# videolan/dav1d

Hardware: AMD Instinct MI355X
Metric: reconstructed luma Mpixels/s (8K 4:2:0 10-bit) on the itx+mc recon path; bit-exact vs C (higher is better)
Workload: dtype int32; 1 GPU; frame_contexts=2, picture_layout=tiled, parity=not checked in this run (bench.py --full checks it)

## Files before the change

### dav1d_amd/csrc/api_recon.hip

```cpp
#include "lists.h"
#include <stdio.h>
#include <stdlib.h>
#include <new>
#include <algorithm>


int recon_fuse_mask(const Dav1dHipContext *c) { return c->recon_fuse & 31; }

extern "C" {

int dav1d_hip_recon_list_create(Dav1dHipContext *c, Dav1dHipReconList **out, const Dav1dHipPicture *geometry,
                                const Dav1dHipMcTask *mc, size_t n_mc, const Dav1dHipCompTask *comp, size_t n_comp,
                                const Dav1dHipItxTask *itx, size_t n_itx) {
    if (!c || !out || !geometry) return -EINVAL;
    *out = nullptr;
    if ((!itx && n_itx) || n_itx > 0xffffffffu) return -EINVAL;
    for (size_t i = 0; i < n_itx; i++) if (!itx_task_ok(itx[i])) return -EINVAL;
    Dav1dHipReconList *l = new (std::nothrow) Dav1dHipReconList();
    if (!l) return -ENOMEM;
    const Dav1dHipItxTask *const itx_all = itx;
    const size_t n_itx_all = n_itx;
    l->inter = nullptr; l->itx = nullptr; l->wide_ok = false;
    for (int k = 0; k < 5; k++) { l->f_tiles[k] = nullptr; l->f_tasks[k] = nullptr; l->f_n[k] = 0; }
    l->f_max_ref = 0;
// ... 92 lines not shown

void dav1d_hip_recon_list_destroy(Dav1dHipContext *c, Dav1dHipReconList *l) {
    if (!l) return;
    if (l->inter) dav1d_hip_inter_list_destroy(c, l->inter);
    if (l->itx) dav1d_hip_itx_list_destroy(c, l->itx);
    hipStreamSynchronize(c->stream);
    for (int k = 0; k < 5; k++) { if (l->f_tiles[k]) hipFree(l->f_tiles[k]); if (l->f_tasks[k]) hipFree(l->f_tasks[k]); }
    delete l;
}

static int recon_list_run_impl(Dav1dHipContext *c, const Dav1dHipReconList *l, const Dav1dHipPicture *dst, const Dav1dHipPicture *refs, int n_refs,
                               int16_t *prep, uint8_t *mask, void *coef, const bool wide, const DevPlanes *dst_twin) {
    if (!c || !l || !dst || !refs) return -EINVAL;
    const int bps = dst->bpc > 8 ? 2 : 1;
    for (int p = 0; p < 3; p++)
        if (l->stride_px[p] && dst->p[p].stride / bps != l->stride_px[p]) return -EINVAL;
    size_t n_paired = 0;
    bool paired_on_side = false;
    int n_ps = 0;
    for (int k = 0; k < 5; k++) n_paired += l->f_n[k];
    if (n_paired) {
        const DevPlanes dp = dev_planes(dst);
        DevPlanes rp[8];
        if (const int rv = checked_ref_planes(c, dst, refs, n_refs, l->f_max_ref, rp)) return rv;
        const bool side = c->concurrent && n_paired >= 16384;
        int rc = 0, lane = 0;
        n_ps = side ? std::max(1, std::min(3, c->recon_pair_streams)) : 0;
        if (side) {
            (void) hipEventRecord(c->ev_fork, c->stream);
            for (int j = 0; j < n_ps; j++) (void) hipStreamWaitEvent(c->side[c->recon_pair_first + j], c->ev_fork, 0);
        }
        for (int k = 4; k >= 0 && !rc; k--)
            if (l->f_n[k]) {
                const bool on_main = side && k == 0;
                rc = dav1d_hip_launch_recon_fused_out(&dp, rp, n_refs, dst->bpc, k, l->f_tiles[k], l->f_tasks[k], (int) l->f_n[k], prep, coef, c->recon_coop_below,
                                                      wide, dst_twin, side && !on_main ? c->side[c->recon_pair_first + lane] : c->stream);
                if (!on_main && n_ps) lane = (lane + 1) % n_ps;
            }
        for (int j = 0; j < n_ps; j++) (void) hipEventRecord(c->ev_pair[j], c->side[c->recon_pair_first + j]);
        if (rc) return rc;
        paired_on_side = side;
        if (!l->inter->mc->n && !l->inter->comp->n && !l->itx->n) {
            for (int j = 0; j < n_ps; j++) (void) hipStreamWaitEvent(c->stream, c->ev_pair[j], 0);
            return 0;
        }
    }
    const Dav1dHipMcList *ml = l->inter->mc;
    const long min_tasks = c->recon_pipeline;
    auto join_paired = [&]() {
        if (paired_on_side) for (int j = 0; j < n_ps; j++) (void) hipStreamWaitEvent(c->stream, c->ev_pair[j], 0);
    };
    if (!dst_twin && (min_tasks < 0 || !c->concurrent || mc_fused_min_bin() < MC_BINS || (long) l->itx->n < min_tasks)) {
        int rc = dav1d_hip_inter_list_run(c, l->inter, dst, refs, n_refs, prep, mask);
        if (!rc) rc = dav1d_hip_itx_list_run(c, l->itx, dst, coef);
        join_paired();
        return rc;
    }
    const DevPlanes dp = dev_planes(dst);
    DevPlanes rp[8];
    if (const int rv = checked_ref_planes(c, dst, refs, n_refs, ml->n ? ml->max_ref : 0, rp)) { join_paired(); return rv; }
    int rc = mc_regroup(c, const_cast<Dav1dHipMcList *>(ml), rp, n_refs);
    if (rc) { join_paired(); return rc; }
    const int n_lanes = paired_on_side ? 1
                      : std::max(1, std::min((int) Dav1dHipContext::N_SIDE, c->recon_lanes));
    hipStream_t sm = c->stream;
    (void) hipEventRecord(c->ev_fork, sm);
    for (int i = 0; i < n_lanes; i++) (void) hipStreamWaitEvent(c->side[i], c->ev_fork, 0);
// ... 154 lines not shown
```

### dav1d_amd/csrc/capi.h

```cpp
#pragma once
#include "common.h"
#include <errno.h>
#include <mutex>
#include <vector>

struct Dav1dHipContext {
    int device;
    hipStream_t stream;
    bool own_stream;
    void *scratch;
    size_t scratch_size;
    enum { N_SIDE = 6 };
    hipStream_t side[N_SIDE];
    hipEvent_t ev_fork, ev_join[N_SIDE];
    hipEvent_t ev_pair[3];
    hipEvent_t ev_bin[16];
    bool concurrent;
    int flow_min_steps;
    int flow_mode;
    int flow_groups;
    int intra_sb;
    int intra_sb_flow;
    int intra_sb_lds;
    int intra_sb_waves;
    long intra_sb_fallbacks;
    int intra_sb_one_below;
    int recon_fuse;
    long recon_pipeline;
    int recon_lanes;
    int chunk_upload;
    int recon_coop_below;
    int post_bands;
    int colour_cells;
    int recon_pair_streams;
    int recon_pair_first;
    hipStream_t pad_streams[8]; int n_pad_streams;
    int ref_twin;
    bool cdef_rows;
    bool cdef_full_copy;
    bool cdef_unit_kernel;
    hipEvent_t ev_t0, ev_t1;
    float last_ms;
    bool last_ms_pending;
    struct Slab { uint8_t *host; size_t cap; };
    std::mutex pool_mtx;
    std::vector<Slab> free_slabs[48];
    struct Arena { uint8_t *dev; size_t cap; };
    std::vector<Arena> free_arenas;
    std::vector<Arena> free_task_bufs;
    std::vector<Dav1dHipPicture> free_pictures;
    size_t arena_hint;
    uint32_t *band_cnt = nullptr, *band_flags = nullptr;
    uint32_t band_seq = 0;
    int chunk_hints;
    int prep_async;
    int chunk_order;
    size_t arena_min;
    size_t uarena_hint = 0;
    size_t carena_hint;
    uint8_t *gather_dev, *segtab_dev;
    size_t gather_cap, segtab_cap;
    uint8_t *pending_slab;
    size_t pending_slab_cap;
    hipStream_t copy_stream;
    hipEvent_t ev_copy;
    hipEvent_t ev_untile;
    hipEvent_t ev_retile;
// ... 347 lines not shown
```

### dav1d_amd/csrc/capi.hip

```cpp
#include "capi.h"

#ifndef RECON_FUSE_DEFAULT
#define RECON_FUSE_DEFAULT 15
#endif
#include <stdlib.h>
#include <string.h>
#include <atomic>
#include <new>
#include <algorithm>
extern "C" void dav1d_hip_note_context_device(int device);

extern "C" {


long long dav1d_hip_live[8];
int dav1d_hip_live_objects(long long out[4]) {
    if (!out) return -EINVAL;
    for (int i = 0; i < 4; i++) out[i] = __atomic_load_n(&dav1d_hip_live[i], __ATOMIC_RELAXED);
    return 0;
}

int dav1d_hip_open(Dav1dHipContext **out, int device, void *stream) {
    if (!out) return -EINVAL;
    *out = nullptr;
    int ndev = 0;
    if (hipGetDeviceCount(&ndev) != hipSuccess || ndev <= 0 || device < 0 || device >= ndev)
        return -ENODEV;
    if (hipSetDevice(device) != hipSuccess) return -ENODEV;
    Dav1dHipContext *c = new (std::nothrow) Dav1dHipContext();
    if (!c) return -ENOMEM;
    c->device = device;
    c->own_stream = stream == nullptr;
    dav1d_hip_note_context_device(device);
    c->scratch = nullptr;
    c->scratch_size = 0;
    if (stream) c->stream = (hipStream_t) stream;
    else if (hipStreamCreate(&c->stream) != hipSuccess) { delete c; return -ENODEV; }
#ifndef DAV1D_HIP_EMU
    {
        hipDeviceProp_t prop;
        if (hipGetDeviceProperties(&prop, device) != hipSuccess || strncmp(prop.gcnArchName, "gfx950", 6)) { delete c; return -ENODEV; }
    }
#endif
    auto env_int = [](const char *name, long dflt) { const char *e = getenv(name); return e ? atol(e) : dflt; };
    c->recon_fuse = (int) env_int("DAV1D_HIP_RECON_FUSE", RECON_FUSE_DEFAULT);
    c->recon_pipeline = env_int("DAV1D_HIP_RECON_PIPELINE", 16384);
    c->recon_lanes = (int) env_int("DAV1D_HIP_RECON_LANES", 1);
    c->chunk_upload = (int) env_int("DAV1D_HIP_CHUNK_UPLOAD", 0);
    c->recon_coop_below = (int) env_int("DAV1D_HIP_RECON_COOP_BELOW", 4096);
    c->post_bands = (int) env_int("DAV1D_HIP_POST_BANDS", 0);
    c->colour_cells = (int) env_int("DAV1D_HIP_COLOUR_CELLS", 0);
    c->ref_twin = (int) env_int("DAV1D_HIP_REF_TWIN", 1);
    c->recon_pair_streams = (int) env_int("DAV1D_HIP_RECON_PAIR_STREAMS", 2);
    static std::atomic<int> n_opened{0};
    const int ctx_index = n_opened.fetch_add(1);
    auto env_list = [&](const char *name, long dflt) {
        const char *e = getenv(name);
        if (!e || !*e) return dflt;
        int n = 1;
        for (const char *q = e; *q; q++) n += *q == ',';
        int want = ctx_index % n;
        const char *q = e;
        while (want-- > 0) q = strchr(q, ',') + 1;
        return atol(q);
    };
    c->recon_pair_first = (int) std::max(1L, std::min(3L, env_list("DAV1D_HIP_RECON_PAIR_FIRST", 2)));
    c->n_pad_streams = (int) std::max(0L, std::min(8L, env_list("DAV1D_HIP_STREAM_PAD", 1)));
    for (int i = 0; i < c->n_pad_streams; i++)
        if (hipStreamCreateWithFlags(&c->pad_streams[i], hipStreamNonBlocking) != hipSuccess) { c->n_pad_streams = i; break; }
    const char *ser = getenv("DAV1D_HIP_SERIAL");
    c->concurrent = !(ser && atoi(ser));
    const char *cu = getenv("DAV1D_HIP_CDEF_UNIT");
    c->cdef_unit_kernel = cu && atoi(cu);
    c->cdef_full_copy = env_int("DAV1D_HIP_FILTER_FULL_COPY", 0) != 0;
    c->cdef_rows = env_int("DAV1D_HIP_CDEF_ROWS", 1) != 0;
    const char *fg = getenv("DAV1D_HIP_FLOW_GROUPS");
    c->flow_groups = fg && atoi(fg) > 0 ? atoi(fg) : 512;
    const char *fm = getenv("DAV1D_HIP_FLOW_MODE");
    c->flow_mode = fm ? atoi(fm) : 0;
    const char *fs = getenv("DAV1D_HIP_FLOW_MIN_STEPS");
    c->flow_min_steps = fs ? atoi(fs) : 200;
    const char *isb = getenv("DAV1D_HIP_INTRA_SB");
    c->intra_sb = isb ? atoi(isb) : 2;
    c->intra_sb_waves = (int) env_int("DAV1D_HIP_INTRA_SB_WAVES", 0);
    c->intra_sb_one_below = (int) env_int("DAV1D_HIP_INTRA_SB_ONE_BELOW", 0);
    c->intra_sb_fallbacks = 0;
// ... 99 lines not shown
    if (!graph) return -EIO;
    Dav1dHipGraph *g = new (std::nothrow) Dav1dHipGraph();
    if (!g) { hipGraphDestroy(graph); return -ENOMEM; }
    g->graph = graph;
    g->nodes = 0;
    (void) hipGraphGetNodes(graph, nullptr, &g->nodes);
    const hipError_t e = hipGraphInstantiate(&g->exec, graph, nullptr, nullptr, 0);
    if (e != hipSuccess) { hipGraphDestroy(graph); delete g; return hip_rc(e); }
    *out = g;
    return 0;
}

int dav1d_hip_graph_launch(Dav1dHipContext *c, const Dav1dHipGraph *g) {
    if (!c || !g) return -EINVAL;
    return hip_rc(hipGraphLaunch(g->exec, c->stream));
}

size_t dav1d_hip_graph_nodes(const Dav1dHipGraph *g) { return g ? g->nodes : 0; }

void dav1d_hip_graph_destroy(Dav1dHipContext *c, Dav1dHipGraph *g) {
    if (!g) return;
    if (c) hipStreamSynchronize(c->stream);
    hipGraphExecDestroy(g->exec);
    hipGraphDestroy(g->graph);
    delete g;
}
int dav1d_hip_get_option(Dav1dHipContext *c, const char *name, long *value) {
    if (!c || !name || !value) return -EINVAL;
    if (!strcmp(name, "intra_sb_fallbacks")) *value = c->intra_sb_fallbacks;
    else if (!strcmp(name, "intra_sb_waves")) *value = c->intra_sb_waves;
    else if (!strcmp(name, "intra_sb_one_below")) *value = c->intra_sb_one_below;
    else if (!strcmp(name, "recon_fuse")) *value = c->recon_fuse;
    else if (!strcmp(name, "recon_pair_streams")) *value = c->recon_pair_streams;
    else if (!strcmp(name, "recon_pair_first")) *value = c->recon_pair_first;
    else if (!strcmp(name, "ref_twin")) *value = c->ref_twin;
    else return -EINVAL;
    return 0;
}
int dav1d_hip_set_option(Dav1dHipContext *c, const char *name, long value) {
    if (!c || !name) return -EINVAL;
    if (!strcmp(name, "recon_fuse")) c->recon_fuse = (int) value;
    else if (!strcmp(name, "recon_pipeline")) c->recon_pipeline = value;
    else if (!strcmp(name, "recon_lanes")) c->recon_lanes = (int) value;
    else if (!strcmp(name, "chunk_upload")) c->chunk_upload = (int) value;
    else if (!strcmp(name, "recon_coop_below")) c->recon_coop_below = (int) value;
    else if (!strcmp(name, "post_bands")) c->post_bands = (int) value;
    else if (!strcmp(name, "colour_cells")) c->colour_cells = value < 0 ? 0 : value > 64 ? 64 : (int) value;
    else if (!strcmp(name, "ref_twin")) c->ref_twin = (int) value;
    else if (!strcmp(name, "recon_pair_streams")) c->recon_pair_streams = (int) value;
    else if (!strcmp(name, "recon_pair_first")) c->recon_pair_first = (int) std::max(1L, std::min(3L, (long) value));
    else if (!strcmp(name, "serial")) c->concurrent = !value;
    else if (!strcmp(name, "cdef_unit")) c->cdef_unit_kernel = value != 0;
    else if (!strcmp(name, "filter_full_copy")) c->cdef_full_copy = value != 0;
    else if (!strcmp(name, "cdef_rows")) c->cdef_rows = value != 0;
    else if (!strcmp(name, "flow_groups")) c->flow_groups = value > 0 ? (int) value : c->flow_groups;
    else if (!strcmp(name, "flow_mode")) c->flow_mode = (int) value;
    else if (!strcmp(name, "flow_min_steps")) c->flow_min_steps = (int) value;
    else if (!strcmp(name, "intra_sb")) c->intra_sb = (int) value;
    else if (!strcmp(name, "intra_sb_waves")) c->intra_sb_waves = value >= 8 ? 8 : value >= 4 ? 4 : value == 1 ? 1 : 0;
    else if (!strcmp(name, "intra_sb_one_below")) c->intra_sb_one_below = value > 0 ? (int) value : 0;
    else if (!strcmp(name, "intra_sb_lds")) c->intra_sb_lds = value != 0;
    else if (!strcmp(name, "intra_sb_flow")) c->intra_sb_flow = value != 0;
    else if (!strcmp(name, "intra_sb_fine")) dav1d_hip_sbw_set_fine(value != 0);
    else if (!strcmp(name, "intra_sb_fail_at")) dav1d_hip_sbw_set_fail_at((int) value);
    else if (!strcmp(name, "prep_async")) c->prep_async = value < 0 ? 0 : value > 2 ? 2 : (int) value;
    else if (!strcmp(name, "chunk_order")) c->chunk_order = value != 0;
    else if (!strcmp(name, "chunk_hints")) c->chunk_hints = value != 0;
    else if (!strcmp(name, "chunk_arena_min")) { if (value < 4096) return -EINVAL; c->arena_min = (size_t) 1 << 12; while (c->arena_min < (size_t) value) c->arena_min <<= 1; c->arena_hint = 0; }
    else return -EINVAL;
    return 0;
}

const char *dav1d_hip_version(void) { return "dav1d_hip 0.1 (gfx950)"; }
float dav1d_hip_last_kernel_ms(Dav1dHipContext *c) {
    if (!c) return 0.f;
    if (c->last_ms_pending) {
        c->last_ms_pending = false;
        c->last_ms = 0.f;
        if (hipEventSynchronize(c->ev_t1) == hipSuccess) (void) hipEventElapsedTime(&c->last_ms, c->ev_t0, c->ev_t1);
    }
    return c->last_ms;
}
// ... 106 lines not shown
```

### dav1d_amd/csrc/itx1d.h

```cpp
#pragma once
#include <hip/hip_runtime.h>
#include "common.h"

namespace itx1d {

__device__ static constexpr int kCos128[65] = {
    4096, 4095, 4091, 4085, 4076, 4065, 4052, 4036, 4017, 3996, 3973, 3948, 3920,
    3889, 3857, 3822, 3784, 3745, 3703, 3659, 3612, 3564, 3513, 3461, 3406, 3349,
    3290, 3229, 3166, 3102, 3035, 2967, 2896, 2824, 2751, 2675, 2598, 2520, 2440,
    2359, 2276, 2191, 2106, 2019, 1931, 1842, 1751, 1660, 1567, 1474, 1380, 1285,
    1189, 1092,  995,  897,  799,  700,  601,  501,  401,  301,  201,  101,    0,
};

__device__ constexpr int ilog2c(int v) { int r = 0; while (v > 1) { v >>= 1; r++; } return r; }
__device__ constexpr int brev(int v, int bits) {
    int r = 0;
    for (int i = 0; i < bits; i++) r |= ((v >> i) & 1) << (bits - 1 - i);
    return r;
}

__device__ __forceinline__ int clampi(int v, int lo, int hi) { return dv::clamp3(v, lo, hi); }

__device__ __forceinline__ int rot(int a, int b, int ka, int kb) {
    const int qa = ka > 2048 ? 1 : ka < -2048 ? -1 : 0;
    const int qb = kb > 2048 ? 1 : kb < -2048 ? -1 : 0;
    const int fa = ka - 4096 * qa, fb = kb - 4096 * qb;
    int acc = 2048;
    if (fb) acc = dv::mad_i24k(b, fb, acc);
    if (fa) acc = dv::mad_i24k(a, fa, acc);
    return (acc >> 12) + qa * a + qb * b;
}
__device__ __forceinline__ int rot45(int v) { return dv::mad_i24k(v, 181, 128) >> 8; }

template <int N>
__device__ __forceinline__ void idct(const int *in, int *out, const int lo, const int hi) {
    if constexpr (N == 2) {
        out[0] = rot45(in[0] + in[1]);
        out[1] = rot45(in[0] - in[1]);
    } else {
        constexpr int M = N / 2;
        int ev[M], e[M], t[M];
#pragma unroll
        for (int i = 0; i < M; i++) ev[i] = in[2 * i];
        idct<M>(ev, e, lo, hi);

        constexpr int bitsA = ilog2c(M / 2);
#pragma unroll
        for (int i = 0; i < M / 2; i++) {
            const int k = 4 * brev(i, bitsA) + 1;
            const int a = k * 64 / N;
            const int c = kCos128[a], s = kCos128[64 - a];
            const int x = in[k], y = in[N - k];
            t[i] = rot(x, y, s, -c);
            t[M - 1 - i] = rot(x, y, c, s);
        }
#pragma unroll
        for (int g = 2; g <= M / 2; g *= 2) {
#pragma unroll
            for (int G = 0; G < M / g; G++) {
#pragma unroll
                for (int i = 0; i < g / 2; i++) {
                    const int p = G * g + i, q = G * g + g - 1 - i;
                    const int u = t[p], v = t[q];
                    if (G & 1) { t[p] = clampi(v - u, lo, hi); t[q] = clampi(v + u, lo, hi); }
                    else       { t[p] = clampi(u + v, lo, hi); t[q] = clampi(u - v, lo, hi); }
                }
            }
            const int nblk = M / (4 * g) > 0 ? M / (4 * g) : 1;
            const int bitsR = ilog2c(nblk);
#pragma unroll
            for (int j = 0; j < M / 2; j++) {
                const int blk = j / (2 * g), o = j % (2 * g);
                if (o < g / 2 || o >= 3 * g / 2) continue;
                const int m = M - 1 - j;
                const int a = (4 * brev(blk, bitsR) + 1) * 64 * g / M;
                const int u = t[j], v = t[m];
                if (a == 32) {
                    t[j] = rot45(v - u);
                    t[m] = rot45(v + u);
                } else {
                    const int c = kCos128[a], s = kCos128[64 - a];
                    if (o < g) { t[j] = rot(v, u, s, -c);  t[m] = rot(v, u, c, s); }
                    else       { t[j] = rot(v, u, -c, -s); t[m] = rot(v, u, s, -c); }
                }
            }
        }
#pragma unroll
        for (int i = 0; i < M; i++) {
            const int u = e[i], v = t[M - 1 - i];
            out[i] = clampi(u + v, lo, hi);
            out[N - 1 - i] = clampi(u - v, lo, hi);
        }
    }
}

__device__ __forceinline__ void iadst4(const int *in, int *out) {
    const int a = in[0], b = in[1], c = in[2], d = in[3];
    using dv::mad_i24k;
    out[0] = (mad_i24k(a, 1321, mad_i24k(b, 3344 - 4096, mad_i24k(c, 3803 - 4096, mad_i24k(d, 2482 - 4096, 2048)))) >> 12)
             + b + c + d;
    out[1] = (mad_i24k(a, 2482 - 4096, mad_i24k(b, 3344 - 4096, mad_i24k(c, -1321, mad_i24k(d, -(3803 - 4096), 2048)))) >> 12)
             + a + b - d;
    out[2] = mad_i24k(a - c + d, 209, 128) >> 8;
    out[3] = (mad_i24k(a, 3803 - 4096, mad_i24k(b, -(3344 - 4096), mad_i24k(c, 2482 - 4096, mad_i24k(d, -1321, 2048)))) >> 12)
             + a - b + c;
}

template <int N>
__device__ __forceinline__ void iadst(const int *in, int *out, const int lo, const int hi) {
    static_assert(N == 8 || N == 16, "adst size");
    int t[N];
#pragma unroll
    for (int i = 0; i < N / 2; i++) {
        const int a = (4 * i + 1) * 32 / N;
        const int c = kCos128[a], s = kCos128[64 - a];
        const int x = in[N - 1 - 2 * i], y = in[2 * i];
        t[2 * i]     = rot(x, y, c, s);
        t[2 * i + 1] = rot(x, y, s, -c);
    }
// ... 68 lines not shown
```

### dav1d_amd/csrc/itx_body.h

```cpp
#pragma once
#include "common.h"
#include "itx1d.h"
#include "av1_scan_dev.h"
#include <type_traits>

namespace {

enum { K_DCT = 0, K_ADST = 1, K_IDENTITY = 2, K_FLIPADST = 3, K_WHT = 4 };

__host__ __device__ constexpr int tx_w(int tx) {
    constexpr int w[19] = { 4, 8, 16, 32, 64, 4, 8, 8, 16, 16, 32, 32, 64, 4, 16, 8, 32, 16, 64 };
    return w[tx];
}
__host__ __device__ constexpr int tx_h(int tx) {
    constexpr int h[19] = { 4, 8, 16, 32, 64, 8, 4, 16, 8, 32, 16, 64, 32, 16, 4, 32, 8, 64, 16 };
    return h[tx];
}
__host__ __device__ constexpr int tx_shift(int tx) {
    constexpr int s[19] = { 0, 1, 2, 2, 2, 0, 0, 1, 1, 1, 1, 1, 1, 1, 1, 2, 2, 2, 2 };
    return s[tx];
}
__host__ __device__ constexpr int cmin(int a, int b) { return a < b ? a : b; }
__host__ __device__ constexpr int cmax(int a, int b) { return a > b ? a : b; }

// ... 252 lines not shown
            dc = (dc + ((1 << SHIFT) >> 1)) >> SHIFT;
            dc = (dc * 181 + 128 + 2048) >> 12;
#pragma unroll
            for (int y = 0; y < H; y++)
                o[y * ostride] = ((pixel) dv::clamp3((int) dpx[y] + dc, 0, bitdepth_max));
        } else {
            int out[H];
            if (TX == 0 && wht) {
                if constexpr (H == 4) itx1d::iwht4(cin, out);
#pragma unroll
                for (int y = 0; y < H; y++)
                    o[y * ostride] = ((pixel) dv::clamp3((int) dpx[y] + out[y], 0, bitdepth_max));
            } else {
                tx1d<H>(k2, cin, col_min, col_max, [&](const int *res) {
                    if (k2 == K_FLIPADST) {
#pragma unroll
                        for (int y = 0; y < H; y++)
                            o[y * ostride] = ((pixel) dv::clamp3((int) dpx[y] + ((res[H - 1 - y] + 8) >> 4), 0, bitdepth_max));
                    } else {
#pragma unroll
                        for (int y = 0; y < H; y++)
                            o[y * ostride] = ((pixel) dv::clamp3((int) dpx[y] + ((res[y] + 8) >> 4), 0, bitdepth_max));
                    }
                });
            }
        }
    }
    DV_PHASE(PH + 3);
    DV_PHASE_WAVE(PH + 4);
}



template <int W, int H, int BPW, typename pixel>
__device__ __forceinline__ void tile_write_out(const pixel *tile, const Dav1dHipItxTask *__restrict__ tasks, const int nb,
                                               const DevPlanes &dst, const DevPlanes &twin, const bool has_twin, const bool raster = true,
                                               const uint32_t task_off = 0, const int task_plane = -1)
{
    constexpr int CP = W < 8 ? W : 8;
    constexpr int CPR = W / CP, PER_BLOCK = H * CPR, NCHK = BPW * PER_BLOCK;
    constexpr int BYTES = CP * (int) sizeof(pixel);
    typedef typename std::conditional<BYTES == 16, uint4, typename std::conditional<BYTES == 8, uint2, uint32_t>::type>::type piece_t;
    static_assert(BYTES == 4 || BYTES == 8 || BYTES == 16, "piece size");
    const int lane = dv::lane_id();
    constexpr int LPBX = 64 / BPW;
    constexpr bool OWN = BPW > 1 && PER_BLOCK == LPBX;
    constexpr bool ONE = BPW > 1 && PER_BLOCK % 64 == 0;
    constexpr bool TWO = BPW > 1 && PER_BLOCK == 32;
    const bool direct = task_plane >= 0 && (OWN || ONE || TWO);
    int bx = 0, by = 0, bpl = 0;
    if (direct) {
        if constexpr (OWN) {
            bpl = task_plane;
            dv::off_to_xy(task_off, bpl == 0 ? dst.stride[0] : bpl == 1 ? dst.stride[1] : dst.stride[2], bx, by);
        }
    } else if (task_plane >= 0) {
        const uint32_t off = BPW == 1 ? task_off : (uint32_t) __shfl((int) task_off, (lane & (BPW - 1)) * LPBX);
        bpl = BPW == 1 ? task_plane : __shfl(task_plane, (lane & (BPW - 1)) * LPBX);
        if (lane < nb) dv::off_to_xy(off, bpl == 0 ? dst.stride[0] : bpl == 1 ? dst.stride[1] : dst.stride[2], bx, by);
    } else if (lane < nb) {
        const Dav1dHipItxTask t = tasks[lane];
        bpl = t.plane;
        dv::off_to_xy(t.dst_off, bpl == 0 ? dst.stride[0] : bpl == 1 ? dst.stride[1] : dst.stride[2], bx, by);
    }
#pragma unroll
    for (int i0 = 0; i0 < NCHK; i0 += 64) {
        const int i = i0 + lane;
        const int b = BPW == 1 ? 0 : (i / PER_BLOCK) & (BPW - 1), rem = i - (i / PER_BLOCK) * PER_BLOCK;
        const int y = rem / CPR, c = rem - y * CPR;
        int x0, y0, pl;
        if constexpr (BPW == 1) { x0 = __builtin_amdgcn_readfirstlane(bx); y0 = __builtin_amdgcn_readfirstlane(by); pl = __builtin_amdgcn_readfirstlane(bpl); }
        else if (direct && OWN) { x0 = bx; y0 = by; pl = bpl; }
        else if (direct && ONE) {
            const int bl = ((i0 / PER_BLOCK) & (BPW - 1)) * LPBX;
            pl = dv::readlane(task_plane, bl);
            dv::off_to_xy((uint32_t) dv::readlane((int) task_off, bl), pl == 0 ? dst.stride[0] : pl == 1 ? dst.stride[1] : dst.stride[2], x0, y0);
        } else if (direct && TWO) {
            const int bl = ((i0 / PER_BLOCK) & (BPW - 1)) * LPBX;
            const bool hi = lane >= 32;
            pl = hi ? dv::readlane(task_plane, bl + LPBX) : dv::readlane(task_plane, bl);
            const uint32_t off = (uint32_t) (hi ? dv::readlane((int) task_off, bl + LPBX) : dv::readlane((int) task_off, bl));
            dv::off_to_xy(off, pl == 0 ? dst.stride[0] : pl == 1 ? dst.stride[1] : dst.stride[2], x0, y0);
        } else { x0 = __shfl(bx, b); y0 = __shfl(by, b); pl = __shfl(bpl, b); }
        if (i >= NCHK || i / PER_BLOCK >= nb) continue;
        const piece_t v = *reinterpret_cast<const piece_t *>(tile + b * itx_tile_stride(W, H) + y * W + c * CP);
#ifdef DV_KO_WRITE
        if (*reinterpret_cast<const uint32_t *>(&v) != 0xfeedbeefu) continue;
#endif
        const int X = x0 + c * CP, Y = y0 + y;
        const int stride = pl == 0 ? dst.stride[0] : pl == 1 ? dst.stride[1] : dst.stride[2];
        pixel *const base = reinterpret_cast<pixel *>(pl == 0 ? dst.data[0] : pl == 1 ? dst.data[1] : dst.data[2]);
        if (raster) *reinterpret_cast<piece_t *>(base + (dv::mul_i24(Y, stride) + X)) = v;
        if (has_twin) {
            pixel *const tb = reinterpret_cast<pixel *>(pl == 0 ? twin.data[0] : pl == 1 ? twin.data[1] : twin.data[2]);
            *reinterpret_cast<piece_t *>(tb + (dv::mul_i24(Y & ~7, stride) + ((X >> 3) << 6) + ((Y & 7) << 3) + (X & 7))) = v;
        }
    }
}

}
// ... 1 lines not shown
```

### dav1d_amd/csrc/recon.hip

```cpp
#define DV_UNIT recon
#include "mc_body.h"
#include "itx_body.h"
#include <string.h>

DV_PHASE_DEFINE(DV_UNIT)
namespace {

#ifndef RECON_WAVES
#define RECON_WAVES 7
#endif
#ifndef RECON_WAVES_8
#define RECON_WAVES_8 7
#endif
#ifndef RECON_WAVES_32
#define RECON_WAVES_32 7
#endif

constexpr int rc_log2(int v) { return v <= 1 ? 0 : 1 + rc_log2(v >> 1); }

template <int CLS> constexpr int recon_waves() {
    constexpr int W = 4 << CLS, TW = mc_cmin(W, 64), TH = mc_cmin(W, 16), TPB = (W / TW) * (W / TH);
    constexpr int LPB = cmax(cmin(W, 32), W), BPW = 64 / LPB, G = 64 / mc_cmin(64, TW * TH / 4);
    return (BPW * TPB + G - 1) / G;
}

template <int CLS, typename pixel, typename coef, bool COOP, bool TILED, bool WIDE>
__global__ __launch_bounds__(COOP ? 64 * recon_waves<CLS>() : 64, COOP ? 1 : CLS == 1 ? RECON_WAVES_8 : CLS == 3 ? RECON_WAVES_32 : RECON_WAVES)
void recon_fused_kernel(const DevPlanes dst, const RefSet refs, const McTile *__restrict__ tiles,
                        const Dav1dHipItxTask *__restrict__ tasks, const int n_blocks,
                        int16_t *__restrict__ prep, coef *__restrict__ cf, const int bitdepth_max, const DevPlanes twin)
{
    constexpr int TX = CLS;
    constexpr int W = 4 << CLS;
    constexpr int TW = mc_cmin(W, 64), TH = mc_cmin(W, 16);
    constexpr int TPB = (W / TW) * (W / TH);
    constexpr int LPB = cmax(cmin(W, 32), W), BPW = 64 / LPB;
    constexpr int G = 64 / mc_cmin(64, TW * TH / 4);
    constexpr int NW = COOP ? recon_waves<CLS>() : 1;
    constexpr int MC_B = (mc_lds_bytes<TW, TH, TILED>() + 15) / 16 * 16, PRED_B = BPW * itx_tile_stride(W, W) * (int) sizeof(pixel);
    constexpr int ITX_B = itx_lds_ints<TX>() * 4;
    constexpr int LDS_B = cmax(NW * MC_B + PRED_B, ITX_B);
    __shared__ uint4 smem[(LDS_B + 15) / 16];
    const int wave = NW == 1 ? 0 : (int) (threadIdx.x >> 6);
    uint4 *const smem_mc = reinterpret_cast<uint4 *>(reinterpret_cast<char *>(smem) + wave * MC_B);
    pixel *const pred = reinterpret_cast<pixel *>(reinterpret_cast<char *>(smem) + NW * MC_B);
    int *const smem_itx = reinterpret_cast<int *>(smem);

    const int group = (int) dv::xcd_chunk_id(blockIdx.x, gridDim.x);
    const int block0 = group * BPW;
    if (block0 >= n_blocks) return;
    DV_PHASE_BEGIN();
    const int nb = dv::imin(BPW, n_blocks - block0);
    const int tile0 = block0 * TPB, ntile = nb * TPB;
#ifdef DV_KO_NOMC
    if (bitdepth_max == 12345)
#endif
    if constexpr (NW == 1) {
        for (int c = 0; c < ntile; c += G) {
            mc_body<TW, TH, pixel, true, TILED>(dst, refs, tiles, tile0 + c, dv::imin(G, ntile - c), prep, bitdepth_max, smem_mc,
                                         pred, tile0, rc_log2(TPB), W, W);
            dv::wave_sync();
        }
    } else {
        const int c = wave * G;
        if (c < ntile)
            mc_body<TW, TH, pixel, true, TILED>(dst, refs, tiles, tile0 + c, dv::imin(G, ntile - c), prep, bitdepth_max, smem_mc,
                                         pred, tile0, rc_log2(TPB), W, W);
        __syncthreads();
        if (wave) return;
    }
    DV_PHASE(768 + CLS * 16 + 0);
    if constexpr (WIDE) {
        uint32_t toff = 0;
        int tpl = 0;
#ifdef DV_KO_NOITX
        if (bitdepth_max == 12345)
#endif
        itx_body<TX, pixel, coef, true, true>(dst, tasks, n_blocks, cf, bitdepth_max, group, smem_itx, pred, false, &toff, &tpl);
        dv::wave_sync();
        DV_PHASE(768 + CLS * 16 + 1);
#ifdef DV_KO_NOOUT
        if (bitdepth_max == 12345)
#endif
        tile_write_out<W, W, BPW, pixel>(pred, tasks + block0, nb, dst, twin, twin.data[0] != nullptr, twin.tiled != 2, toff, tpl);
        DV_PHASE(768 + CLS * 16 + 2);
    } else {
        itx_body<TX, pixel, coef, true>(dst, tasks, n_blocks, cf, bitdepth_max, group, smem_itx, pred);
        DV_PHASE(768 + CLS * 16 + 1);
    }
    DV_PHASE_WAVE(768 + CLS * 16 + 3);
}

template <int CLS, typename pixel, typename coef, bool TILED, bool WIDE>
void launch_cls(const DevPlanes &dst, const RefSet &refs, const McTile *tiles, const Dav1dHipItxTask *tasks, const int n,
                int16_t *prep, coef *cf, const int bitdepth_max, const int coop_below, const DevPlanes &twin, hipStream_t stream)
{
    constexpr int W = 4 << CLS, LPB = cmax(cmin(W, 32), W), BPW = 64 / LPB;
    const int groups = (n + BPW - 1) / BPW;
#ifndef DV_LEAN
    if (recon_waves<CLS>() > 1 && groups < coop_below)
        hipLaunchKernelGGL((recon_fused_kernel<CLS, pixel, coef, true, TILED, WIDE>), dim3(groups), dim3(64 * recon_waves<CLS>()), 0, stream,
                           dst, refs, tiles, tasks, n, prep, cf, bitdepth_max, twin);
    else
#endif
        hipLaunchKernelGGL((recon_fused_kernel<CLS, pixel, coef, false, TILED, WIDE>), dim3(groups), dim3(64), 0, stream,
                           dst, refs, tiles, tasks, n, prep, cf, bitdepth_max, twin);
}

template <typename pixel, typename coef, bool TILED, bool WIDE>
hipError_t launch_any(const int cls, const DevPlanes &dst, const RefSet &refs, const McTile *tiles, const Dav1dHipItxTask *tasks,
                      const int n, int16_t *prep, coef *cf, const int bitdepth_max, const int coop_below, const DevPlanes &twin, hipStream_t stream)
{
    switch (cls) {
    case 0: launch_cls<0, pixel, coef, TILED, WIDE>(dst, refs, tiles, tasks, n, prep, cf, bitdepth_max, coop_below, twin, stream); break;
    case 1: launch_cls<1, pixel, coef, TILED, WIDE>(dst, refs, tiles, tasks, n, prep, cf, bitdepth_max, coop_below, twin, stream); break;
    case 2: launch_cls<2, pixel, coef, TILED, WIDE>(dst, refs, tiles, tasks, n, prep, cf, bitdepth_max, coop_below, twin, stream); break;
    case 3: launch_cls<3, pixel, coef, TILED, WIDE>(dst, refs, tiles, tasks, n, prep, cf, bitdepth_max, coop_below, twin, stream); break;
    case 4: launch_cls<4, pixel, coef, TILED, WIDE>(dst, refs, tiles, tasks, n, prep, cf, bitdepth_max, coop_below, twin, stream); break;
    default: return hipErrorInvalidValue;
    }
    return hipGetLastError();
}

template <typename pixel, typename coef>
hipError_t launch_variant(const bool tiled, const bool wide, const int cls, const DevPlanes &dst, const RefSet &refs, const McTile *tiles,
                          const Dav1dHipItxTask *tasks, const int n, int16_t *prep, coef *cf, const int bitdepth_max, const int coop_below,
                          const DevPlanes &twin, hipStream_t st)
{
#ifdef DV_LEAN
    if (!tiled || !wide || sizeof(pixel) != 2) return hipErrorInvalidValue;
    if constexpr (sizeof(pixel) == 2) return launch_any<pixel, coef, true, true>(cls, dst, refs, tiles, tasks, n, prep, cf, bitdepth_max, coop_below, twin, st);
    else return hipErrorInvalidValue;
#else
    if (tiled) return wide ? launch_any<pixel, coef, true, true>(cls, dst, refs, tiles, tasks, n, prep, cf, bitdepth_max, coop_below, twin, st)
                           : launch_any<pixel, coef, true, false>(cls, dst, refs, tiles, tasks, n, prep, cf, bitdepth_max, coop_below, twin, st);
    return wide ? launch_any<pixel, coef, false, true>(cls, dst, refs, tiles, tasks, n, prep, cf, bitdepth_max, coop_below, twin, st)
                : launch_any<pixel, coef, false, false>(cls, dst, refs, tiles, tasks, n, prep, cf, bitdepth_max, coop_below, twin, st);
#endif
}
// ... 30 lines not shown
```

Measured before the change: 155,800 Mpixels/s.

## Add two-wave 64x64 recon-pair kernel splitting IDCT even/odd halves across waves

Adds a dedicated two-wave workgroup path for 64x64 inter+residual pairs (class 4). Each wave predicts half the tiles, then the 64-point row and column IDCTs are split so one wave computes the even half and the other the odd half, exchanging results through LDS. The kernel previously ran these as single-wave work with heavy per-lane register pressure. The change also turns on fuse bit 4 by default so this class is fused, and runs class 4 on the main stream instead of a side stream. It adds more barriers and LDS traffic per block.

Result: no change. 155,000 Mpixels/s (-0.5%).

```diff
diff --git a/dav1d_amd/csrc/api_recon.hip b/dav1d_amd/csrc/api_recon.hip
--- a/dav1d_amd/csrc/api_recon.hip
+++ b/dav1d_amd/csrc/api_recon.hip
@@ -148,7 +148,7 @@
         }
         for (int k = 4; k >= 0 && !rc; k--)
             if (l->f_n[k]) {
-                const bool on_main = side && k == 0;
+                const bool on_main = side && (k == 0 || (k == 4 && c->recon_pair64_main));
                 rc = dav1d_hip_launch_recon_fused_out(&dp, rp, n_refs, dst->bpc, k, l->f_tiles[k], l->f_tasks[k], (int) l->f_n[k], prep, coef, c->recon_coop_below,
                                                       wide, dst_twin, side && !on_main ? c->side[c->recon_pair_first + lane] : c->stream);
                 if (!on_main && n_ps) lane = (lane + 1) % n_ps;
diff --git a/dav1d_amd/csrc/capi.h b/dav1d_amd/csrc/capi.h
--- a/dav1d_amd/csrc/capi.h
+++ b/dav1d_amd/csrc/capi.h
@@ -33,6 +33,7 @@
     int post_bands;
     int colour_cells;
     int recon_pair_streams;
+    int recon_pair64_main;
     int recon_pair_first;
     hipStream_t pad_streams[8]; int n_pad_streams;
     int ref_twin;
diff --git a/dav1d_amd/csrc/capi.hip b/dav1d_amd/csrc/capi.hip
--- a/dav1d_amd/csrc/capi.hip
+++ b/dav1d_amd/csrc/capi.hip
@@ -1,7 +1,7 @@
 #include "capi.h"
 
 #ifndef RECON_FUSE_DEFAULT
-#define RECON_FUSE_DEFAULT 15
+#define RECON_FUSE_DEFAULT 31
 #endif
 #include <stdlib.h>
 #include <string.h>
@@ -52,6 +52,7 @@
     c->colour_cells = (int) env_int("DAV1D_HIP_COLOUR_CELLS", 0);
     c->ref_twin = (int) env_int("DAV1D_HIP_REF_TWIN", 1);
     c->recon_pair_streams = (int) env_int("DAV1D_HIP_RECON_PAIR_STREAMS", 2);
+    c->recon_pair64_main = (int) env_int("DAV1D_HIP_RECON_PAIR64_MAIN", 1);
     static std::atomic<int> n_opened{0};
     const int ctx_index = n_opened.fetch_add(1);
     auto env_list = [&](const char *name, long dflt) {
@@ -217,6 +218,7 @@
     else if (!strcmp(name, "intra_sb_one_below")) *value = c->intra_sb_one_below;
     else if (!strcmp(name, "recon_fuse")) *value = c->recon_fuse;
     else if (!strcmp(name, "recon_pair_streams")) *value = c->recon_pair_streams;
+    else if (!strcmp(name, "recon_pair64_main")) *value = c->recon_pair64_main;
     else if (!strcmp(name, "recon_pair_first")) *value = c->recon_pair_first;
     else if (!strcmp(name, "ref_twin")) *value = c->ref_twin;
     else return -EINVAL;
@@ -233,6 +235,7 @@
     else if (!strcmp(name, "colour_cells")) c->colour_cells = value < 0 ? 0 : value > 64 ? 64 : (int) value;
     else if (!strcmp(name, "ref_twin")) c->ref_twin = (int) value;
     else if (!strcmp(name, "recon_pair_streams")) c->recon_pair_streams = (int) value;
+    else if (!strcmp(name, "recon_pair64_main")) c->recon_pair64_main = value != 0;
     else if (!strcmp(name, "recon_pair_first")) c->recon_pair_first = (int) std::max(1L, std::min(3L, (long) value));
     else if (!strcmp(name, "serial")) c->concurrent = !value;
     else if (!strcmp(name, "cdef_unit")) c->cdef_unit_kernel = value != 0;
diff --git a/dav1d_amd/csrc/itx1d.h b/dav1d_amd/csrc/itx1d.h
--- a/dav1d_amd/csrc/itx1d.h
+++ b/dav1d_amd/csrc/itx1d.h
@@ -33,58 +33,73 @@
 __device__ __forceinline__ int rot45(int v) { return dv::mad_i24k(v, 181, 128) >> 8; }
 
 template <int N>
+__device__ __forceinline__ void idct(const int *in, int *out, const int lo, const int hi);
+
+template <int N>
+__device__ __forceinline__ void idct_even(const int *in, int *e, const int lo, const int hi) {
+    constexpr int M = N / 2;
+    int ev[M];
+#pragma unroll
+    for (int i = 0; i < M; i++) ev[i] = in[2 * i];
+    idct<M>(ev, e, lo, hi);
+}
+
+template <int N>
+__device__ __forceinline__ void idct_odd(const int *in, int *t, const int lo, const int hi) {
+    constexpr int M = N / 2;
+    constexpr int bitsA = ilog2c(M / 2);
+#pragma unroll
+    for (int i = 0; i < M / 2; i++) {
+        const int k = 4 * brev(i, bitsA) + 1;
+        const int a = k * 64 / N;
+        const int c = kCos128[a], s = kCos128[64 - a];
+        const int x = in[k], y = in[N - k];
+        t[i] = rot(x, y, s, -c);
+        t[M - 1 - i] = rot(x, y, c, s);
+    }
+#pragma unroll
+    for (int g = 2; g <= M / 2; g *= 2) {
+#pragma unroll
+        for (int G = 0; G < M / g; G++) {
+#pragma unroll
+            for (int i = 0; i < g / 2; i++) {
+                const int p = G * g + i, q = G * g + g - 1 - i;
+                const int u = t[p], v = t[q];
+                if (G & 1) { t[p] = clampi(v - u, lo, hi); t[q] = clampi(v + u, lo, hi); }
+                else       { t[p] = clampi(u + v, lo, hi); t[q] = clampi(u - v, lo, hi); }
+            }
+        }
+        const int nblk = M / (4 * g) > 0 ? M / (4 * g) : 1;
+        const int bitsR = ilog2c(nblk);
+#pragma unroll
+        for (int j = 0; j < M / 2; j++) {
+            const int blk = j / (2 * g), o = j % (2 * g);
+            if (o < g / 2 || o >= 3 * g / 2) continue;
+            const int m = M - 1 - j;
+            const int a = (4 * brev(blk, bitsR) + 1) * 64 * g / M;
+            const int u = t[j], v = t[m];
+            if (a == 32) {
+                t[j] = rot45(v - u);
+                t[m] = rot45(v + u);
+            } else {
+                const int c = kCos128[a], s = kCos128[64 - a];
+                if (o < g) { t[j] = rot(v, u, s, -c);  t[m] = rot(v, u, c, s); }
+                else       { t[j] = rot(v, u, -c, -s); t[m] = rot(v, u, s, -c); }
+            }
+        }
+    }
+}
+
+template <int N>
 __device__ __forceinline__ void idct(const int *in, int *out, const int lo, const int hi) {
     if constexpr (N == 2) {
         out[0] = rot45(in[0] + in[1]);
         out[1] = rot45(in[0] - in[1]);
     } else {
         constexpr int M = N / 2;
-        int ev[M], e[M], t[M];
-#pragma unroll
-        for (int i = 0; i < M; i++) ev[i] = in[2 * i];
-        idct<M>(ev, e, lo, hi);
-
-        constexpr int bitsA = ilog2c(M / 2);
-#pragma unroll
-        for (int i = 0; i < M / 2; i++) {
-            const int k = 4 * brev(i, bitsA) + 1;
-            const int a = k * 64 / N;
-            const int c = kCos128[a], s = kCos128[64 - a];
-            const int x = in[k], y = in[N - k];
-            t[i] = rot(x, y, s, -c);
-            t[M - 1 - i] = rot(x, y, c, s);
-        }
-#pragma unroll
-        for (int g = 2; g <= M / 2; g *= 2) {
-#pragma unroll
-            for (int G = 0; G < M / g; G++) {
-#pragma unroll
-                for (int i = 0; i < g / 2; i++) {
-                    const int p = G * g + i, q = G * g + g - 1 - i;
-                    const int u = t[p], v = t[q];
-                    if (G & 1) { t[p] = clampi(v - u, lo, hi); t[q] = clampi(v + u, lo, hi); }
-                    else       { t[p] = clampi(u + v, lo, hi); t[q] = clampi(u - v, lo, hi); }
-                }
-            }
-            const int nblk = M / (4 * g) > 0 ? M / (4 * g) : 1;
-            const int bitsR = ilog2c(nblk);
-#pragma unroll
-            for (int j = 0; j < M / 2; j++) {
-                const int blk = j / (2 * g), o = j % (2 * g);
-                if (o < g / 2 || o >= 3 * g / 2) continue;
-                const int m = M - 1 - j;
-                const int a = (4 * brev(blk, bitsR) + 1) * 64 * g / M;
-                const int u = t[j], v = t[m];
-                if (a == 32) {
-                    t[j] = rot45(v - u);
-                    t[m] = rot45(v + u);
-                } else {
-                    const int c = kCos128[a], s = kCos128[64 - a];
-                    if (o < g) { t[j] = rot(v, u, s, -c);  t[m] = rot(v, u, c, s); }
-                    else       { t[j] = rot(v, u, -c, -s); t[m] = rot(v, u, s, -c); }
-                }
-            }
-        }
+        int e[M], t[M];
+        idct_even<N>(in, e, lo, hi);
+        idct_odd<N>(in, t, lo, hi);
 #pragma unroll
         for (int i = 0; i < M; i++) {
             const int u = e[i], v = t[M - 1 - i];
diff --git a/dav1d_amd/csrc/itx_body.h b/dav1d_amd/csrc/itx_body.h
--- a/dav1d_amd/csrc/itx_body.h
+++ b/dav1d_amd/csrc/itx_body.h
@@ -308,11 +308,12 @@
 
 
 
-template <int W, int H, int BPW, typename pixel>
+template <int W, int H, int BPW, typename pixel, int NWV = 1>
 __device__ __forceinline__ void tile_write_out(const pixel *tile, const Dav1dHipItxTask *__restrict__ tasks, const int nb,
                                                const DevPlanes &dst, const DevPlanes &twin, const bool has_twin, const bool raster = true,
-                                               const uint32_t task_off = 0, const int task_plane = -1)
+                                               const uint32_t task_off = 0, const int task_plane = -1, const int wv = 0)
 {
+    static_assert(NWV == 1 || BPW == 1, "several waves share the tile of ONE block");
     constexpr int CP = W < 8 ? W : 8;
     constexpr int CPR = W / CP, PER_BLOCK = H * CPR, NCHK = BPW * PER_BLOCK;
     constexpr int BYTES = CP * (int) sizeof(pixel);
@@ -340,8 +341,8 @@
         dv::off_to_xy(t.dst_off, bpl == 0 ? dst.stride[0] : bpl == 1 ? dst.stride[1] : dst.stride[2], bx, by);
     }
 #pragma unroll
-    for (int i0 = 0; i0 < NCHK; i0 += 64) {
-        const int i = i0 + lane;
+    for (int i0 = 0; i0 < NCHK; i0 += 64 * NWV) {
+        const int i = i0 + (NWV == 1 ? 0 : wv * 64) + lane;
         const int b = BPW == 1 ? 0 : (i / PER_BLOCK) & (BPW - 1), rem = i - (i / PER_BLOCK) * PER_BLOCK;
         const int y = rem / CPR, c = rem - y * CPR;
         int x0, y0, pl;
diff --git a/dav1d_amd/csrc/recon.hip b/dav1d_amd/csrc/recon.hip
--- a/dav1d_amd/csrc/recon.hip
+++ b/dav1d_amd/csrc/recon.hip
@@ -1,6 +1,7 @@
 #define DV_UNIT recon
 #include "mc_body.h"
 #include "itx_body.h"
+#include "recon_pair64.h"
 #include <string.h>
 
 DV_PHASE_DEFINE(DV_UNIT)
@@ -19,6 +20,7 @@
 constexpr int rc_log2(int v) { return v <= 1 ? 0 : 1 + rc_log2(v >> 1); }
 
 template <int CLS> constexpr int recon_waves() {
+    if (CLS == 4) return 2;
     constexpr int W = 4 << CLS, TW = mc_cmin(W, 64), TH = mc_cmin(W, 16), TPB = (W / TW) * (W / TH);
     constexpr int LPB = cmax(cmin(W, 32), W), BPW = 64 / LPB, G = 64 / mc_cmin(64, TW * TH / 4);
     return (BPW * TPB + G - 1) / G;
@@ -41,6 +43,14 @@
     constexpr int ITX_B = itx_lds_ints<TX>() * 4;
     constexpr int LDS_B = cmax(NW * MC_B + PRED_B, ITX_B);
     __shared__ uint4 smem[(LDS_B + 15) / 16];
+    if constexpr (CLS == 4) {
+        static_assert(COOP && LDS_B == Pair64<pixel, coef, TILED>::LDS_B, "64x64 pairs: the two-wave workgroup");
+        const int block = (int) dv::xcd_chunk_id(blockIdx.x, gridDim.x);
+        if (block >= n_blocks) return;
+        DV_PHASE_BEGIN();
+        recon_pair64_body<pixel, coef, TILED, WIDE>(dst, refs, tiles, tasks, block, prep, cf, bitdepth_max, twin, smem);
+        DV_PHASE_WAVE(768 + CLS * 16 + 3);
+    } else {
     const int wave = NW == 1 ? 0 : (int) (threadIdx.x >> 6);
     uint4 *const smem_mc = reinterpret_cast<uint4 *>(reinterpret_cast<char *>(smem) + wave * MC_B);
     pixel *const pred = reinterpret_cast<pixel *>(reinterpret_cast<char *>(smem) + NW * MC_B);
@@ -89,6 +99,7 @@
         DV_PHASE(768 + CLS * 16 + 1);
     }
     DV_PHASE_WAVE(768 + CLS * 16 + 3);
+    }
 }
 
 template <int CLS, typename pixel, typename coef, bool TILED, bool WIDE>
@@ -97,14 +108,19 @@
 {
     constexpr int W = 4 << CLS, LPB = cmax(cmin(W, 32), W), BPW = 64 / LPB;
     const int groups = (n + BPW - 1) / BPW;
-#ifndef DV_LEAN
-    if (recon_waves<CLS>() > 1 && groups < coop_below)
+    if constexpr (CLS == 4) {
         hipLaunchKernelGGL((recon_fused_kernel<CLS, pixel, coef, true, TILED, WIDE>), dim3(groups), dim3(64 * recon_waves<CLS>()), 0, stream,
                            dst, refs, tiles, tasks, n, prep, cf, bitdepth_max, twin);
-    else
+    } else {
+#ifndef DV_LEAN
+        if (recon_waves<CLS>() > 1 && groups < coop_below)
+            hipLaunchKernelGGL((recon_fused_kernel<CLS, pixel, coef, true, TILED, WIDE>), dim3(groups), dim3(64 * recon_waves<CLS>()), 0, stream,
+                               dst, refs, tiles, tasks, n, prep, cf, bitdepth_max, twin);
+        else
 #endif
-        hipLaunchKernelGGL((recon_fused_kernel<CLS, pixel, coef, false, TILED, WIDE>), dim3(groups), dim3(64), 0, stream,
-                           dst, refs, tiles, tasks, n, prep, cf, bitdepth_max, twin);
+            hipLaunchKernelGGL((recon_fused_kernel<CLS, pixel, coef, false, TILED, WIDE>), dim3(groups), dim3(64), 0, stream,
+                               dst, refs, tiles, tasks, n, prep, cf, bitdepth_max, twin);
+    }
 }
 
 template <typename pixel, typename coef, bool TILED, bool WIDE>
diff --git a/dav1d_amd/csrc/recon_pair64.h b/dav1d_amd/csrc/recon_pair64.h
--- /dev/null
+++ b/dav1d_amd/csrc/recon_pair64.h
@@ -0,0 +1,175 @@
+#pragma once
+#include "mc_body.h"
+#include "itx_body.h"
+
+namespace {
+
+template <typename pixel, typename coef, bool TILED>
+struct Pair64 {
+    static constexpr int W = 64, SH = 32, TS = W + 1;
+    static constexpr int MC_B = (mc_lds_bytes<64, 16, TILED>() + 15) / 16 * 16;
+    static constexpr int PRED_B = itx_tile_stride(W, W) * (int) sizeof(pixel);
+    static constexpr int ROW_B = SH * TS * 4, SLAB_B = SH * SH * (int) sizeof(coef), XCH_B = 2 * 16 * 64 * 4;
+    static constexpr int LDS_B = 2 * MC_B + PRED_B;
+    static_assert(ROW_B % 16 == 0 && ROW_B + SLAB_B <= 2 * MC_B && XCH_B <= 2 * MC_B, "the transform's buffers fit the prediction windows");
+};
+
+template <typename pixel, typename coef, bool TILED, bool WIDE>
+__device__ __forceinline__ void recon_pair64_body(const DevPlanes &dst, const RefSet &refs, const McTile *__restrict__ tiles,
+                                                  const Dav1dHipItxTask *__restrict__ tasks, const int block, int16_t *__restrict__ prep,
+                                                  coef *__restrict__ cf, const int bitdepth_max, const DevPlanes &twin, uint4 *smem)
+{
+    typedef Pair64<pixel, coef, TILED> P;
+    constexpr int W = 64, SH = 32, TS = P::TS, SHIFT = tx_shift(4);
+    constexpr bool HBD = sizeof(pixel) == 2;
+    constexpr int NCH = P::SLAB_B / 16, NV = (NCH + 127) / 128;
+    const int tid = (int) threadIdx.x, lane = tid & 63;
+    const int wave = __builtin_amdgcn_readfirstlane(tid >> 6);
+
+    uint4 *const smem_mc = reinterpret_cast<uint4 *>(reinterpret_cast<char *>(smem) + wave * P::MC_B);
+    pixel *const pred = reinterpret_cast<pixel *>(reinterpret_cast<char *>(smem) + 2 * P::MC_B);
+    int *const tmp = reinterpret_cast<int *>(smem);
+    coef *const slab = reinterpret_cast<coef *>(reinterpret_cast<char *>(smem) + P::ROW_B);
+    int *const xch = reinterpret_cast<int *>(smem);
+
+    const Dav1dHipItxTask t = tasks[__builtin_amdgcn_readfirstlane(block)];
+    const bool dconly = t.txtp == 0 && t.eob < 1;
+    const bool packed = t.flags & DAV1D_HIP_ITX_PACKED;
+    coef *const gcf = cf + t.cf_off;
+    const int nch = dconly || packed ? 0 : (((int) t.rsv[0] | ((int) t.rsv[1] << 8)) * (int) sizeof(coef) + 15) >> 4;
+    const int tile0 = block * 4;
+#pragma unroll 1
+    for (int j = 0; j < 2; j++) {
+        mc_body<64, 16, pixel, true, TILED>(dst, refs, tiles, tile0 + 2 * wave + j, 1, prep, bitdepth_max, smem_mc, pred, tile0, 2, W, W);
+        dv::wave_sync();
+    }
+    int4 v[NV];
+#pragma unroll
+    for (int k = 0; k < NV; k++) {
+        v[k] = make_int4(0, 0, 0, 0);
+        if (tid + k * 128 < nch) v[k] = reinterpret_cast<const int4 *>(gcf)[tid + k * 128];
+    }
+    int dc = 0;
+    if (dconly) dc = gcf[0];
+    __syncthreads();
+
+    const int st0 = dst.stride[0], st1 = dst.stride[1], st2 = dst.stride[2];
+    void *const dp0 = dst.data[0], *const dp1 = dst.data[1], *const dp2 = dst.data[2];
+    const int stride = t.plane == 0 ? st0 : t.plane == 1 ? st1 : st2;
+    pixel *const d = reinterpret_cast<pixel *>(t.plane == 0 ? dp0 : t.plane == 1 ? dp1 : dp2) + t.dst_off + lane;
+    pixel *const pc = pred + lane;
+    auto emit = [&](const int y, const int res) {
+        const pixel px = (pixel) dv::clamp3((int) pc[y * W] + res, 0, bitdepth_max);
+        if (WIDE) pc[y * W] = px;
+        else d[y * stride] = px;
+    };
+
+    if (dconly) {
+        if (tid == 0 && !packed) gcf[0] = 0;
+        dc = (dc * 181 + 128) >> 8;
+        dc = (dc + ((1 << SHIFT) >> 1)) >> SHIFT;
+        dc = (dc * 181 + 128 + 2048) >> 12;
+#pragma unroll
+        for (int y = 0; y < 32; y++) emit(wave * 32 + y, dc);
+    } else {
+#pragma unroll
+        for (int k = 0; k < NV; k++) {
+            const int i = tid + k * 128;
+            if (i < NCH) reinterpret_cast<int4 *>(slab)[i] = v[k];
+            if (i < nch) reinterpret_cast<int4 *>(gcf)[i] = make_int4(0, 0, 0, 0);
+        }
+        if (packed) {
+            __syncthreads();
+            const int cls = (t.txtp == 11 || t.txtp == 13 || t.txtp == 15) ? 1 : (t.txtp == 10 || t.txtp == 12 || t.txtp == 14) ? 2 : 0;
+            const uint16_t *const scan = av1_scans + av1_scan_off[4];
+            for (int i = tid; i <= t.eob; i += 128) {
+                const int rc = cls == 0 ? (int) scan[i] : cls == 1 ? i : ((i & (SH - 1)) * SH + (i >> 5));
+                slab[rc] = gcf[i];
+            }
+        }
+        __syncthreads();
+
+        int row_min, col_min;
+        if (HBD) {
+            row_min = (int) ((unsigned) ~bitdepth_max << 7);
+            col_min = (int) ((unsigned) ~bitdepth_max << 5);
+        } else {
+            row_min = col_min = -32768;
+        }
+        const int row_max = ~row_min, col_max = ~col_min;
+
+        if (lane < SH) {
+            int in[W], h[32];
+#pragma unroll
+            for (int x = 0; x < W; x++) in[x] = 0;
+            if (wave == 0) {
+#pragma unroll
+                for (int x = 0; x < SH; x += 2) in[x] = slab[x * SH + lane];
+                itx1d::idct_even<64>(in, h, row_min, row_max);
+#pragma unroll
+                for (int i = 0; i < 32; i++) tmp[lane * TS + i] = h[i];
+            } else {
+#pragma unroll
+                for (int x = 1; x < SH; x += 2) in[x] = slab[x * SH + lane];
+                itx1d::idct_odd<64>(in, h, row_min, row_max);
+#pragma unroll
+                for (int i = 0; i < 32; i++) tmp[lane * TS + 32 + i] = h[i];
+            }
+        }
+        __syncthreads();
+        {
+            const int rnd = (1 << SHIFT) >> 1;
+#pragma unroll
+            for (int k = 0; k < SH * 32 / 128; k++) {
+                const int p = tid + k * 128, r = p >> 5, i = p & 31;
+                const int a = tmp[r * TS + i], b = tmp[r * TS + 63 - i];
+                const int o0 = dv::clamp3(a + b, row_min, row_max), o1 = dv::clamp3(a - b, row_min, row_max);
+                tmp[r * TS + i] = dv::clamp3((o0 + rnd) >> SHIFT, col_min, col_max);
+                tmp[r * TS + 63 - i] = dv::clamp3((o1 + rnd) >> SHIFT, col_min, col_max);
+            }
+        }
+        __syncthreads();
+
+        int h[32];
+        {
+            int in[W];
+#pragma unroll
+            for (int y = 0; y < W; y++) in[y] = 0;
+            if (wave == 0) {
+#pragma unroll
+                for (int y = 0; y < SH; y += 2) in[y] = tmp[y * TS + lane];
+            } else {
+#pragma unroll
+                for (int y = 1; y < SH; y += 2) in[y] = tmp[y * TS + lane];
+            }
+            __syncthreads();
+            if (wave == 0) itx1d::idct_even<64>(in, h, col_min, col_max);
+            else itx1d::idct_odd<64>(in, h, col_min, col_max);
+        }
+#pragma unroll
+        for (int j = 0; j < 16; j++) xch[(wave * 16 + j) * 64 + lane] = h[16 + j];
+        __syncthreads();
+        if (wave == 0) {
+#pragma unroll
+            for (int i = 0; i < 16; i++) {
+                const int tv = xch[(16 + 15 - i) * 64 + lane];
+                emit(i, (dv::clamp3(h[i] + tv, col_min, col_max) + 8) >> 4);
+                emit(63 - i, (dv::clamp3(h[i] - tv, col_min, col_max) + 8) >> 4);
+            }
+        } else {
+#pragma unroll
+            for (int i = 16; i < 32; i++) {
+                const int ev = xch[(i - 16) * 64 + lane];
+                emit(i, (dv::clamp3(ev + h[31 - i], col_min, col_max) + 8) >> 4);
+                emit(63 - i, (dv::clamp3(ev - h[31 - i], col_min, col_max) + 8) >> 4);
+            }
+        }
+    }
+
+    if constexpr (WIDE) {
+        __syncthreads();
+        tile_write_out<W, W, 1, pixel, 2>(pred, tasks + block, 1, dst, twin, twin.data[0] != nullptr, twin.tiled != 2, t.dst_off, t.plane, wave);
+    }
+}
+
+}
```
